# NagabhushanSN95/ViP-NeRF

Measured on AMD Instinct MI355X. Metric: train_rays_per_sec, higher is better.
Workload: dtype f32; 1 GPU; BASELINE configs[1]: fern geometry (NDC), 2 views, 4096 rays/iter/GPU x (64+128) samples, coarse+fine 8x256 MLP, V=1 secondary view(s), losses MSE+Visibility+VisibilityPrior, Adam; rays generated and random numbers drawn on device; rays_per_gpu=4096, global_rays=4096, parallelism=ray-sharded dp1, gemm_arithmetic=fp32

## Files before the change

### vip-nerf_amd/csrc/vipnerf_knobs.h

```cpp
#pragma once

#define VN_KNOB_LIST(X)                                                                                                                   \
                                                    \
    X(VN_BF16_NARROW_DEFAULT) X(VN_FP32_NARROW_DEFAULT)                                                                                   \
                     \
    X(VN_STAGE_CHUNKS) X(VN_SPLIT_FMA_MIX) X(VN_INTERLEAVE) X(VN_SKEW) X(VN_DMA_MODE) X(VN_DMA_ISSUERS) X(VN_F16_PRESPLIT) X(VN_DEFER_STORES)             \
    X(VN_STORE_GROUP_A) X(VN_STORE_GROUP_B) X(VN_F32_PERSISTENT) X(VN_F32_EVAL_ROTATE) X(VN_F32B_CONV_GROUP) X(VN_DMA_ROT_WAVES) X(VN_F32_DMA_ISSUERS)                                                              \
        \
    X(VN_BF16_H16) X(VN_T16) X(VN_T16_X4) X(VN_T16_NT) X(VN_PT2_SPREAD) X(VN_PT2_SKEW) X(VN_PT2_G) X(VN_PT2_D)                  \
    X(VN_PT2_TRAIN_KEEP) X(VN_PT2_EVAL_KEEP) X(VN_PT2_FAST_PE)                                                                                              \
                                                                           \
    X(VN_WGRAD_SIGMA_FUSED) X(VN_WGRAD_VIEW_FUSED) X(VN_WGRAD_HEADS_FUSED) X(VN_WGRAD_LATE_LOAD) X(VN_WGRAD_LATE_STORE) X(VN_WGRAD_STORE_SKEW) X(VN_WGRAD_FAST) X(VN_WGRAD_BIAS_WK0) X(VN_WGRAD_VECFRAG) X(VN_WGRAD_PREFETCH) X(VN_WGRAD_DMA) X(VN_WGRAD_W8) X(VN_WGRAD_PIPE) X(VN_WGRAD_ONE_ROUND) X(VN_WGRAD_ROUNDS) X(VN_WG16_BIG_WM) X(VN_WG16_BIG_WN)        \
    X(VN_WG16_BIG_NB) X(VN_WG16_HYBRID) X(VN_WG16_SIGMA_FUSED) X(VN_WG16_DMA_PIECES) X(VN_WG16_THIN_HYBRID) X(VN_WG16_BIG_SLOTS) X(VN_WG16_VIEW_FUSED) X(VN_WG16_VIEW_WN)          \
                                                                                                         \
    X(VN_ADAM_FMA_MASK)

#ifndef VN_BF16_NARROW_DEFAULT
#define VN_BF16_NARROW_DEFAULT 1
#endif
#ifndef VN_FP32_NARROW_DEFAULT
#define VN_FP32_NARROW_DEFAULT 1
#endif
#ifndef VN_STAGE_CHUNKS
#define VN_STAGE_CHUNKS 64
#endif
#ifndef VN_SPLIT_FMA_MIX
#define VN_SPLIT_FMA_MIX 1
#endif
#ifndef VN_INTERLEAVE
#define VN_INTERLEAVE 1
#endif
#ifndef VN_SKEW
#define VN_SKEW 0
#endif
#ifndef VN_DMA_MODE
#define VN_DMA_MODE 1
#endif
#ifndef VN_DMA_ISSUERS
#define VN_DMA_ISSUERS 1
#endif
#ifndef VN_F16_PRESPLIT
#define VN_F16_PRESPLIT 1
#endif
#ifndef VN_DEFER_STORES
#define VN_DEFER_STORES 1
#endif
#ifndef VN_STORE_GROUP_A
#define VN_STORE_GROUP_A 6
#endif
#ifndef VN_STORE_GROUP_B
#define VN_STORE_GROUP_B 12
#endif
#ifndef VN_F32_PERSISTENT
#define VN_F32_PERSISTENT 1
#endif
#ifndef VN_F32_EVAL_ROTATE
#define VN_F32_EVAL_ROTATE 1
#endif
#ifndef VN_WGRAD_SIGMA_FUSED
#define VN_WGRAD_SIGMA_FUSED 1
#endif
#ifndef VN_WGRAD_VIEW_FUSED
#define VN_WGRAD_VIEW_FUSED 1
#endif
#ifndef VN_F32_DMA_ISSUERS
#define VN_F32_DMA_ISSUERS 4
#endif
#ifndef VN_DMA_ROT_WAVES
#define VN_DMA_ROT_WAVES 4
#endif
#ifndef VN_F32B_CONV_GROUP
#define VN_F32B_CONV_GROUP 2
#endif
#ifndef VN_BF16_H16
#define VN_BF16_H16 1
#endif
#ifndef VN_T16
#define VN_T16 1
#endif
#ifndef VN_T16_X4
#define VN_T16_X4 1
#endif
#ifndef VN_T16_NT
#define VN_T16_NT 1
#endif
#ifndef VN_PT2_SPREAD
#define VN_PT2_SPREAD 4
#endif
#ifndef VN_PT2_SKEW
#define VN_PT2_SKEW 0
#endif
#ifndef VN_PT2_G
#define VN_PT2_G 1
#endif
#ifndef VN_PT2_D
#define VN_PT2_D 2
#endif
#ifndef VN_PT2_TRAIN_KEEP
#define VN_PT2_TRAIN_KEEP 0
#endif
#ifndef VN_PT2_EVAL_KEEP
#define VN_PT2_EVAL_KEEP 1
#endif
#ifndef VN_PT2_FAST_PE
#define VN_PT2_FAST_PE 1
#endif
#ifndef VN_WGRAD_LATE_LOAD
#define VN_WGRAD_LATE_LOAD 2
#endif
#ifndef VN_WGRAD_LATE_STORE
#define VN_WGRAD_LATE_STORE 12
#endif
#ifndef VN_WGRAD_HEADS_FUSED
#define VN_WGRAD_HEADS_FUSED 1
#endif
#ifndef VN_WGRAD_STORE_SKEW
#define VN_WGRAD_STORE_SKEW 2
#endif
#ifndef VN_WGRAD_FAST
#define VN_WGRAD_FAST 1
#endif
#ifndef VN_WGRAD_BIAS_WK0
#define VN_WGRAD_BIAS_WK0 1
#endif
#ifndef VN_WGRAD_VECFRAG
#define VN_WGRAD_VECFRAG 1
#endif
#ifndef VN_WGRAD_PREFETCH
#define VN_WGRAD_PREFETCH 1
#endif
#ifndef VN_WGRAD_DMA
#define VN_WGRAD_DMA 0
#endif
#ifndef VN_WGRAD_W8
#define VN_WGRAD_W8 2
#endif
#ifndef VN_WGRAD_PIPE
#define VN_WGRAD_PIPE 1
#endif
#ifndef VN_WGRAD_ONE_ROUND
#define VN_WGRAD_ONE_ROUND 1
#endif
#ifndef VN_WGRAD_ROUNDS
#define VN_WGRAD_ROUNDS 1
#endif
#ifndef VN_WG16_BIG_WM
#define VN_WG16_BIG_WM 2
#endif
#ifndef VN_WG16_BIG_WN
#define VN_WG16_BIG_WN 4
#endif
#ifndef VN_WG16_BIG_NB
#define VN_WG16_BIG_NB 4
#endif
#ifndef VN_WG16_HYBRID
#define VN_WG16_HYBRID 1
#endif
#ifndef VN_WG16_SIGMA_FUSED
#define VN_WG16_SIGMA_FUSED 1
#endif
#ifndef VN_WG16_DMA_PIECES
#define VN_WG16_DMA_PIECES 2
#endif
#ifndef VN_WG16_THIN_HYBRID
#define VN_WG16_THIN_HYBRID 0
#endif
#ifndef VN_WG16_VIEW_FUSED
#define VN_WG16_VIEW_FUSED 1
#endif
#ifndef VN_WG16_VIEW_WN
#define VN_WG16_VIEW_WN 2
#endif
#ifndef VN_WG16_BIG_SLOTS
#define VN_WG16_BIG_SLOTS 256
#endif
#ifndef VN_ADAM_FMA_MASK
#define VN_ADAM_FMA_MASK 7
#endif

#define VN_KNOB_STR2(x) #x
#define VN_KNOB_STR(x) VN_KNOB_STR2(x)
#define VN_KNOB_ITEM(name) " " #name "=" VN_KNOB_STR(name)
#if defined(VN_EXP)
#define VN_EXP_STR "VN_EXP=" VN_KNOB_STR(VN_EXP)
#define VN_EXP_VALUE (VN_EXP)
#else
#define VN_EXP_STR "VN_EXP=unset"
#define VN_EXP_VALUE (-1)
#endif
#define VN_BUILD_INFO_KNOBS VN_EXP_STR VN_KNOB_LIST(VN_KNOB_ITEM)
```

### vip-nerf_amd/csrc/vipnerf_mlp_fwd_f32.hip

```cpp
#include "vipnerf_bf16n.h"
#include "vipnerf_mlp.h"
#include "vipnerf_mlp_pt2.h"

namespace vn {

TS_DECL(g_f32f_timeline);
#define TSFF(tag) TS_AT(g_f32f_timeline, tag)

typedef BnPlan<2> PLFF;

template <bool SAVE>
__device__ __forceinline__ void fwd_conv_kstep(const floatx4 *xr, f32q (*bin)[2], int s, unsigned *mk, bool sig, float *sg, const float *wsig) {
#pragma unroll
    for (int u = 0; u < 2; ++u) {
        const int t = 2 * s + u;
        floatx4 x;
#pragma unroll
        for (int r = 0; r < 4; ++r) x[r] = SAVE ? relu_bits(xr[t][r], 0) : fmaxf(xr[t][r], 0.f);
        if (SAVE) mk[t >> 3] = push_nibble(mk[t >> 3], positive_nibble(x));
        if (sig) {
            const float4 w4 = *(const float4 *)(wsig + 16 * t);
            sg[0] = fmaf(w4.x, x[0], sg[0]); sg[1] = fmaf(w4.y, x[1], sg[1]);
            sg[2] = fmaf(w4.z, x[2], sg[2]); sg[3] = fmaf(w4.w, x[3], sg[3]);
        }
        bin[s][u].v = x;
    }
}

template <bool SAVE, bool CONV>
struct F32FwdMid {
    float *dst; int64_t p; int q, wave, s0;
    f32q (*bin)[2];
    const floatx4 *xr;
    unsigned *mk;
    bool sig; float *sg; const float *wsig;
    uint2 *mask_dst;
    template <int g, int NG> static constexpr bool active() {
        return (SAVE && (g == VN_STORE_GROUP_A || g == VN_STORE_GROUP_B)) || (CONV && g == VN_F32B_CONV_GROUP);
    }
    template <int g, int NG>
    __device__ __forceinline__ void at() const {
        if (CONV && g == VN_F32B_CONV_GROUP) {
            fwd_conv_kstep<SAVE>(xr, bin, s0 + 2, mk, sig, sg, wsig);
            fwd_conv_kstep<SAVE>(xr, bin, s0 + 3, mk, sig, sg, wsig);
            if (SAVE && s0 == 4 && !EXP_NO_STORES) *mask_dst = make_uint2(mk[0], mk[1]);
        }
        if (SAVE && (g == VN_STORE_GROUP_A || g == VN_STORE_GROUP_B) && (g == VN_STORE_GROUP_A) == (wave < 4) && !EXP_NO_STORES) {
#pragma unroll
            for (int s = s0; s < s0 + 2; ++s) {
                store_tile16(dst, p, W, q, 2 * s, bin[s][0].v);
                store_tile16(dst, p, W, q, 2 * s + 1, bin[s][1].v);
            }
        }
    }
};

template <bool SAVE>
__global__ __launch_bounds__(PLFF::WG) void k_mlp_fwd_f32(MlpFwdArgs a) {
    typedef PLFF PL;
    typedef f32q FR;
    extern __shared__ __attribute__((aligned(16))) float lds[];
    float *res = lds;
    float *stage_buf = lds + PL::R_TOTAL_PAD;
    const float *rf = res + PL::R_F32;

    const int tid = threadIdx.x, lane = tid & 63, wave = tid >> 6;
    const int q = lane >> 4, j = lane & 15;
    const int64_t p_raw = (int64_t)blockIdx.x * MLP_PTS_PER_WG + wave * 16 + j;
    const bool valid = p_raw < a.src.P;
    const int64_t p = valid ? p_raw : a.src.P - 1;

    TS_INIT();
    TSFF(TS_ENTRY);
    typename std::conditional<SAVE || VN_F32_EVAL_ROTATE, typename StreamOlder<PL>::type, typename StreamShared<PL>::type>::type ws;
    ws.start(a.packed + PL::PK_FWD, PL::F_STAGES, stage_buf, lane, wave);
    {
        const float4 *g4 = (const float4 *)(a.packed + PL::PK_RES);
        float4 *l4 = (float4 *)res;
        for (int i = tid; i < PL::R_TOTAL_PAD / 4; i += PL::WG) l4[i] = g4[i];
    }
    float pe[2][8];
    {
        PointCtx pc0;
        load_point(a.src, p, pc0);
        encode_x16(pc0.x, q, pe);
    }
    if (SAVE && valid && !EXP_NO_PE) store_x16(a.acts + a.al.pex + (size_t)p * DPE_PAD, q, pe);
    FR bpe[2][2];
#pragma unroll
    for (int s = 0; s < 2; ++s) split8<2>(pe[s], bpe[s]);

    FR bin[8][2];
    floatx4 acc[16], xr[16];
    unsigned mk[2] = {0u, 0u};
    float sg[4] = {0.f, 0.f, 0.f, 0.f};
    const float *wsig = rf + PL::N_WSIG + 4 * q;

    __syncthreads();
    TSFF(TS_RESIDENT);

    {
        const float *bias = rf + PL::N_BIAS + 4 * q;
#pragma unroll
        for (int t = 0; t < 16; ++t) { const float4 b4 = *(const float4 *)(bias + 16 * t); acc[t][0] = b4.x; acc[t][1] = b4.y; acc[t][2] = b4.z; acc[t][3] = b4.w; }
        TSFF(TS_PRE);
        const float *st = ws.wait();
        TSFF(TS_POST);
        gemm_stage_bf<16, PL::KSB, 2>(st, lane, acc, bpe, 0, ws);
        TSFF(TS_END);
#pragma unroll
        for (int t = 0; t < 16; ++t) xr[t] = acc[t];
    }

#pragma unroll 1
    for (int layer = 1; layer <= 8; ++layer) {
        const float *bias = rf + (layer < 8 ? PL::N_BIAS + layer * W : PL::N_BFEAT) + 4 * q;
#pragma unroll
        for (int t = 0; t < 16; ++t) { const float4 b4 = *(const float4 *)(bias + 16 * t); acc[t][0] = b4.x; acc[t][1] = b4.y; acc[t][2] = b4.z; acc[t][3] = b4.w; }
        TSFF(TS_EPI_A);
        const bool sig = layer == 8;
        float *hdst = SAVE ? a.acts + a.al.h[layer - 1] : nullptr;
        uint2 *mdst = SAVE ? (uint2 *)(a.acts + a.al.hm[layer - 1] + ((size_t)p * 4 + q) * 2) : nullptr;
        mk[0] = 0u; mk[1] = 0u;
        fwd_conv_kstep<SAVE>(xr, bin, 0, mk, sig, sg, wsig);
        fwd_conv_kstep<SAVE>(xr, bin, 1, mk, sig, sg, wsig);
        TSFF(TS_EPI_B);
#pragma unroll
        for (int jj = 0; jj < PL::ST_256; ++jj) {
            TSFF(TS_PRE);
            const float *st = SAVE ? (jj == 0 ? ws.template wait<4, 0>(layer == 1 || layer == 6) : ws.template wait<4>()) : ws.wait();
            TSFF(TS_POST);
            if (jj + 1 < PL::ST_256) {
                F32FwdMid<SAVE, true> mid{hdst, p, q, wave, 2 * jj, bin, xr, mk, sig, sg, wsig, mdst};
                gemm_stage_bf<16, PL::KSB, 2>(st, lane, acc, bin, PL::KSB * jj, ws, mid);
            } else {
                F32FwdMid<SAVE, false> mid{hdst, p, q, wave, 2 * jj, bin, xr, mk, sig, sg, wsig, mdst};
                gemm_stage_bf<16, PL::KSB, 2>(st, lane, acc, bin, PL::KSB * jj, ws, mid);
            }
            TSFF(TS_END);
        }
        if (layer == SKIP_LAYER) {
            TSFF(TS_PRE);
            const float *st = SAVE ? ws.template wait<4>() : ws.wait();
            TSFF(TS_POST);
            gemm_stage_bf<16, PL::KSB, 2>(st, lane, acc, bpe, 0, ws);
            TSFF(TS_END);
        }
#pragma unroll
        for (int t = 0; t < 16; ++t) xr[t] = acc[t];
        TSFF(15);
    }

    {
        float s = (sg[0] + sg[1]) + (sg[2] + sg[3]);
        s += __shfl_xor(s, 16, 64);
        s += __shfl_xor(s, 32, 64);
        const float sigma_raw = s + rf[PL::N_BHEAD];
        float nz = 0.f;
        if (a.ns.noise) nz = a.ns.noise[p];
        else if (a.ns.device_rng) nz = rng_normal(a.ns.seed, a.ns.offset, a.ns.stream, noise_index(a.ns, a.src, p));
        const float sgm = fmaxf(__fadd_rn(sigma_raw, __fmul_rn(nz, a.ns.std)), 0.f);
        if (valid && q == 0) a.sigma[p] = sgm;
    }

#pragma unroll
    for (int s = 0; s < 8; ++s) {
        bin[s][0].v = xr[2 * s]; bin[s][1].v = xr[2 * s + 1];
        if (SAVE && !EXP_NO_EXTRAS) {
            store_tile16(a.acts + a.al.feat, p, W, q, 2 * s, xr[2 * s]);
            store_tile16(a.acts + a.al.feat, p, W, q, 2 * s + 1, xr[2 * s + 1]);
        }
    }
    PointCtx pc;
    load_point(a.src, p, pc);
    floatx4 vb[8];
#pragma unroll
    for (int t = 0; t < 8; ++t) {
        const float4 b4 = *(const float4 *)(rf + PL::N_BVIEW + 16 * t + 4 * q);
        vb[t][0] = b4.x; vb[t][1] = b4.y; vb[t][2] = b4.z; vb[t][3] = b4.w;
    }
#pragma unroll
    for (int jj = 0; jj < PL::ST_VIEW_F; ++jj) {
        TSFF(TS_PRE);
        const float *st = SAVE ? (jj == 0 ? ws.template wait<20>() : ws.template wait<0>()) : ws.wait();
        TSFF(TS_POST);
        gemm_stage_bf<8, PL::KSV, 2>(st, lane, vb, bin, PL::KSV * jj, ws);
        TSFF(TS_VIEW);
    }
    stream_end(ws);
    TSFF(16);

#pragma unroll 1
    for (int dsel = 0; dsel <= a.src.V; ++dsel) {
        float dir[3];
        if (dsel == 0) { dir[0] = pc.dir[0]; dir[1] = pc.dir[1]; dir[2] = pc.dir[2]; }
        else secondary_dir(a.src, pc, dsel - 1, dir);
        TSFF(10);
        float ped[1][8];
        encode_d16(dir, q, ped);
        FR bpd[1][2];
        split8<2>(ped[0], bpd[0]);
        floatx4 g[8];
#pragma unroll
        for (int t = 0; t < 8; ++t) g[t] = vb[t];
        { NoStream none; gemm_stage_bf<8, 1, 2>(res + PL::R_DIRW, lane, g, bpd, 0, none); }
#pragma unroll
        for (int t = 0; t < 8; ++t)
#pragma unroll
            for (int r = 0; r < 4; ++r) g[t][r] = relu_lo<SAVE>(g[t][r], 0.f);
        TSFF(12);
        if (SAVE) {
            if (!EXP_NO_EXTRAS) {
#pragma unroll
                for (int t = 0; t < 8; ++t) store_tile16(a.acts + a.al.g[dsel], p, WV, q, t, g[t]);
                unsigned gmb = 0u;
#pragma unroll
                for (int t = 0; t < 8; ++t) gmb = push_nibble(gmb, positive_nibble(g[t]));
                ((unsigned *)(a.acts + a.al.gm[dsel]))[(size_t)p * 4 + q] = gmb;
            }
            if (valid && !EXP_NO_PE) store_d16(a.acts + a.al.ped[dsel] + (size_t)p * DVE_PAD, q, ped);
        }
        TSFF(13);
        float qv[4];
#pragma unroll
        for (int c = 0; c < 4; ++c) {
            const float *wo = rf + PL::N_WOUT + c * WV + 4 * q;
            float s0 = 0.f, s1 = 0.f;
#pragma unroll
            for (int t = 0; t < 8; ++t) {
                const float4 w4 = *(const float4 *)(wo + 16 * t);
                s0 = fmaf(w4.x, g[t][0], s0);
                s1 = fmaf(w4.y, g[t][1], s1);
                s0 = fmaf(w4.z, g[t][2], s0);
                s1 = fmaf(w4.w, g[t][3], s1);
            }
            float s = s0 + s1;
            s += __shfl_xor(s, 16, 64);
            s += __shfl_xor(s, 32, 64);
            qv[c] = sigmoidf_(s + rf[PL::N_BHEAD + 1 + c]);
        }
        if (valid && q == 0) {
            if (dsel == 0) {
                a.rgb[3 * p + 0] = qv[0]; a.rgb[3 * p + 1] = qv[1]; a.rgb[3 * p + 2] = qv[2];
                a.vis[p] = qv[3];
            } else {
                a.vis2[p * a.src.V + (dsel - 1)] = qv[3];
            }
        }
        TSFF(14);
    }
    TSFF(TS_LAST);
}

#if defined(VN_EXP) && VN_EXP == 50
extern "C" int vipnerf_exp_timeline_f32f(unsigned long long *out, int n) {
    return (int)hipMemcpyFromSymbol(out, HIP_SYMBOL(g_f32f_timeline), sizeof(unsigned long long) * (n < 2048 ? n : 2048));
}
#endif

template <bool SAVE>
static int launch_one_f32(const MlpFwdArgs &a, unsigned grid, hipStream_t st) {
    const size_t lds = (size_t)PLFF::LDS_F * sizeof(float);
    VN_HIP(hipFuncSetAttribute((const void *)k_mlp_fwd_f32<SAVE>, hipFuncAttributeMaxDynamicSharedMemorySize, (int)lds));
    hipLaunchKernelGGL(k_mlp_fwd_f32<SAVE>, dim3(grid), dim3(PLFF::WG), lds, st, a);
    VN_HIP(hipGetLastError());
    return VIPNERF_OK;
}

int launch_mlp_fwd_f32(const MlpFwdArgs &a, hipStream_t st) {
    if (a.src.P <= 0) return VIPNERF_OK;
    const unsigned grid = (unsigned)((a.src.P + MLP_PTS_PER_WG - 1) / MLP_PTS_PER_WG);
    return a.acts ? launch_one_f32<true>(a, grid, st) : launch_one_f32<false>(a, grid, st);
}

}
```

Before: 150,100 rays/s.

## Make f32 MLP forward kernel persistent over tiles and add optional early conversion

The f32 forward MLP kernel now loops over multiple point tiles per workgroup, and the grid is capped at the persistent grid size for the training (SAVE) path. Resident weights are then loaded into LDS once per workgroup instead of once per tile, and the weight stream runs across tiles. An optional, default-off knob moves the ReLU/convert step of each layer's output into the tail of the last GEMM stage. The persistent loop adds per-tile index recomputation and asm barriers to keep register pressure down, and it may reduce parallelism if there are too few tiles.

```diff
diff --git a/vip-nerf_amd/csrc/vipnerf_knobs.h b/vip-nerf_amd/csrc/vipnerf_knobs.h
--- a/vip-nerf_amd/csrc/vipnerf_knobs.h
+++ b/vip-nerf_amd/csrc/vipnerf_knobs.h
@@ -5,7 +5,7 @@
     X(VN_BF16_NARROW_DEFAULT) X(VN_FP32_NARROW_DEFAULT)                                                                                   \
                      \
     X(VN_STAGE_CHUNKS) X(VN_SPLIT_FMA_MIX) X(VN_INTERLEAVE) X(VN_SKEW) X(VN_DMA_MODE) X(VN_DMA_ISSUERS) X(VN_F16_PRESPLIT) X(VN_DEFER_STORES)             \
-    X(VN_STORE_GROUP_A) X(VN_STORE_GROUP_B) X(VN_F32_PERSISTENT) X(VN_F32_EVAL_ROTATE) X(VN_F32B_CONV_GROUP) X(VN_DMA_ROT_WAVES) X(VN_F32_DMA_ISSUERS)                                                              \
+    X(VN_STORE_GROUP_A) X(VN_STORE_GROUP_B) X(VN_F32_PERSISTENT) X(VN_F32_FWD_PERSISTENT) X(VN_F32_EARLY_CONV) X(VN_F32_EVAL_ROTATE) X(VN_F32B_CONV_GROUP) X(VN_DMA_ROT_WAVES) X(VN_F32_DMA_ISSUERS)                                                              \
         \
     X(VN_BF16_H16) X(VN_T16) X(VN_T16_X4) X(VN_T16_NT) X(VN_PT2_SPREAD) X(VN_PT2_SKEW) X(VN_PT2_G) X(VN_PT2_D)                  \
     X(VN_PT2_TRAIN_KEEP) X(VN_PT2_EVAL_KEEP) X(VN_PT2_FAST_PE)                                                                                              \
@@ -53,6 +53,12 @@
 #endif
 #ifndef VN_F32_PERSISTENT
 #define VN_F32_PERSISTENT 1
+#endif
+#ifndef VN_F32_FWD_PERSISTENT
+#define VN_F32_FWD_PERSISTENT 1
+#endif
+#ifndef VN_F32_EARLY_CONV
+#define VN_F32_EARLY_CONV 0
 #endif
 #ifndef VN_F32_EVAL_ROTATE
 #define VN_F32_EVAL_ROTATE 1
diff --git a/vip-nerf_amd/csrc/vipnerf_mlp_fwd_f32.hip b/vip-nerf_amd/csrc/vipnerf_mlp_fwd_f32.hip
--- a/vip-nerf_amd/csrc/vipnerf_mlp_fwd_f32.hip
+++ b/vip-nerf_amd/csrc/vipnerf_mlp_fwd_f32.hip
@@ -56,29 +56,63 @@
 };
 
 template <bool SAVE>
+struct F32FwdTail {
+    const floatx4 *acc;
+    f32q (*bin)[2];
+    unsigned *mk;
+    bool on, sig; float *sg; const float *wsig;
+    template <int g, int NG> static constexpr bool active() { return g > NG / 2; }
+    template <int g, int NG>
+    __device__ __forceinline__ void at() const {
+        static_assert(NG == 16, "a stage of 2 k-steps x 16 tiles in groups of two tiles");
+        if (on) fwd_conv_kstep<SAVE>(acc, bin, g - NG / 2 - 1, mk, sig, sg, wsig);
+    }
+};
+template <typename M1, typename M2>
+struct MidPair {
+    M1 m1; M2 m2;
+    template <int g, int NG> static constexpr bool active() { return M1::template active<g, NG>() || M2::template active<g, NG>(); }
+    template <int g, int NG>
+    __device__ __forceinline__ void at() const {
+        if (M1::template active<g, NG>()) m1.template at<g, NG>();
+        if (M2::template active<g, NG>()) m2.template at<g, NG>();
+    }
+};
+
+template <bool SAVE>
 __global__ __launch_bounds__(PLFF::WG) void k_mlp_fwd_f32(MlpFwdArgs a) {
     typedef PLFF PL;
     typedef f32q FR;
+    constexpr bool EC = VN_F32_EARLY_CONV != 0;
     extern __shared__ __attribute__((aligned(16))) float lds[];
     float *res = lds;
     float *stage_buf = lds + PL::R_TOTAL_PAD;
     const float *rf = res + PL::R_F32;
 
-    const int tid = threadIdx.x, lane = tid & 63, wave = tid >> 6;
-    const int q = lane >> 4, j = lane & 15;
-    const int64_t p_raw = (int64_t)blockIdx.x * MLP_PTS_PER_WG + wave * 16 + j;
-    const bool valid = p_raw < a.src.P;
-    const int64_t p = valid ? p_raw : a.src.P - 1;
+    const int tid = threadIdx.x, wave = __builtin_amdgcn_readfirstlane(tid >> 6);
+    const int64_t n_tiles = (a.src.P + MLP_PTS_PER_WG - 1) / MLP_PTS_PER_WG;
+    const int my_tiles = (int)((n_tiles - blockIdx.x + gridDim.x - 1) / gridDim.x);
 
     TS_INIT();
     TSFF(TS_ENTRY);
     typename std::conditional<SAVE || VN_F32_EVAL_ROTATE, typename StreamOlder<PL>::type, typename StreamShared<PL>::type>::type ws;
-    ws.start(a.packed + PL::PK_FWD, PL::F_STAGES, stage_buf, lane, wave);
+    ws.start(a.packed + PL::PK_FWD, PL::F_STAGES, stage_buf, tid & 63, wave, my_tiles);
     {
         const float4 *g4 = (const float4 *)(a.packed + PL::PK_RES);
         float4 *l4 = (float4 *)res;
         for (int i = tid; i < PL::R_TOTAL_PAD / 4; i += PL::WG) l4[i] = g4[i];
     }
+#pragma unroll 1
+    for (int tile_k = 0; tile_k < my_tiles; ++tile_k) {
+    int lane = tid & 63;
+    asm volatile("" : "+v"(lane));
+    int q = lane >> 4, j = lane & 15;
+    const float *wsig = rf + PL::N_WSIG + 4 * q;
+    int64_t tile_p0 = ((int64_t)blockIdx.x + (int64_t)tile_k * gridDim.x) * MLP_PTS_PER_WG + wave * 16, P = a.src.P;
+    asm volatile("" : "+s"(tile_p0), "+s"(P));
+    bool valid = tile_p0 + j < P;
+    int64_t p = valid ? tile_p0 + j : P - 1;
+
     float pe[2][8];
     {
         PointCtx pc0;
@@ -94,9 +128,8 @@
     floatx4 acc[16], xr[16];
     unsigned mk[2] = {0u, 0u};
     float sg[4] = {0.f, 0.f, 0.f, 0.f};
-    const float *wsig = rf + PL::N_WSIG + 4 * q;
-
-    __syncthreads();
+
+    if (tile_k == 0) __syncthreads();
     TSFF(TS_RESIDENT);
 
     {
@@ -106,32 +139,52 @@
         TSFF(TS_PRE);
         const float *st = ws.wait();
         TSFF(TS_POST);
-        gemm_stage_bf<16, PL::KSB, 2>(st, lane, acc, bpe, 0, ws);
+        if (EC) {
+            F32FwdTail<SAVE> tl{acc, bin, mk, true, false, sg, wsig};
+            gemm_stage_bf<16, PL::KSB, 2>(st, lane, acc, bpe, 0, ws, tl);
+        } else {
+            gemm_stage_bf<16, PL::KSB, 2>(st, lane, acc, bpe, 0, ws);
+        }
         TSFF(TS_END);
-#pragma unroll
-        for (int t = 0; t < 16; ++t) xr[t] = acc[t];
+        if (!EC) {
+#pragma unroll
+            for (int t = 0; t < 16; ++t) xr[t] = acc[t];
+        }
     }
 
 #pragma unroll 1
     for (int layer = 1; layer <= 8; ++layer) {
         const float *bias = rf + (layer < 8 ? PL::N_BIAS + layer * W : PL::N_BFEAT) + 4 * q;
-#pragma unroll
-        for (int t = 0; t < 16; ++t) { const float4 b4 = *(const float4 *)(bias + 16 * t); acc[t][0] = b4.x; acc[t][1] = b4.y; acc[t][2] = b4.z; acc[t][3] = b4.w; }
-        TSFF(TS_EPI_A);
         const bool sig = layer == 8;
         float *hdst = SAVE ? a.acts + a.al.h[layer - 1] : nullptr;
         uint2 *mdst = SAVE ? (uint2 *)(a.acts + a.al.hm[layer - 1] + ((size_t)p * 4 + q) * 2) : nullptr;
-        mk[0] = 0u; mk[1] = 0u;
-        fwd_conv_kstep<SAVE>(xr, bin, 0, mk, sig, sg, wsig);
-        fwd_conv_kstep<SAVE>(xr, bin, 1, mk, sig, sg, wsig);
-        TSFF(TS_EPI_B);
+        if (EC) {
+            fwd_conv_kstep<SAVE>(acc, bin, 7, mk, sig, sg, wsig);
+            if (SAVE && !EXP_NO_STORES) *mdst = make_uint2(mk[0], mk[1]);
+            mk[0] = 0u; mk[1] = 0u;
+#pragma unroll
+            for (int t = 0; t < 16; ++t) { const float4 b4 = *(const float4 *)(bias + 16 * t); acc[t][0] = b4.x; acc[t][1] = b4.y; acc[t][2] = b4.z; acc[t][3] = b4.w; }
+            TSFF(TS_EPI_B);
+        } else {
+#pragma unroll
+            for (int t = 0; t < 16; ++t) { const float4 b4 = *(const float4 *)(bias + 16 * t); acc[t][0] = b4.x; acc[t][1] = b4.y; acc[t][2] = b4.z; acc[t][3] = b4.w; }
+            TSFF(TS_EPI_A);
+            mk[0] = 0u; mk[1] = 0u;
+            fwd_conv_kstep<SAVE>(xr, bin, 0, mk, sig, sg, wsig);
+            fwd_conv_kstep<SAVE>(xr, bin, 1, mk, sig, sg, wsig);
+            TSFF(TS_EPI_B);
+        }
 #pragma unroll
         for (int jj = 0; jj < PL::ST_256; ++jj) {
             TSFF(TS_PRE);
             const float *st = SAVE ? (jj == 0 ? ws.template wait<4, 0>(layer == 1 || layer == 6) : ws.template wait<4>()) : ws.wait();
             TSFF(TS_POST);
             if (jj + 1 < PL::ST_256) {
-                F32FwdMid<SAVE, true> mid{hdst, p, q, wave, 2 * jj, bin, xr, mk, sig, sg, wsig, mdst};
+                F32FwdMid<SAVE, !EC> mid{hdst, p, q, wave, 2 * jj, bin, xr, mk, sig, sg, wsig, mdst};
+                gemm_stage_bf<16, PL::KSB, 2>(st, lane, acc, bin, PL::KSB * jj, ws, mid);
+            } else if (EC) {
+                MidPair<F32FwdMid<SAVE, false>, F32FwdTail<SAVE>> mid{{hdst, p, q, wave, 2 * jj, bin, xr, mk, sig, sg, wsig, mdst},
+                                                                     {acc, bin, mk, layer != SKIP_LAYER && layer < 8, layer + 1 == 8, sg, wsig}};
                 gemm_stage_bf<16, PL::KSB, 2>(st, lane, acc, bin, PL::KSB * jj, ws, mid);
             } else {
                 F32FwdMid<SAVE, false> mid{hdst, p, q, wave, 2 * jj, bin, xr, mk, sig, sg, wsig, mdst};
@@ -143,13 +196,29 @@
             TSFF(TS_PRE);
             const float *st = SAVE ? ws.template wait<4>() : ws.wait();
             TSFF(TS_POST);
-            gemm_stage_bf<16, PL::KSB, 2>(st, lane, acc, bpe, 0, ws);
+            if (EC) {
+                F32FwdTail<SAVE> tl{acc, bin, mk, true, false, sg, wsig};
+                gemm_stage_bf<16, PL::KSB, 2>(st, lane, acc, bpe, 0, ws, tl);
+            } else {
+                gemm_stage_bf<16, PL::KSB, 2>(st, lane, acc, bpe, 0, ws);
+            }
             TSFF(TS_END);
         }
+        if (!EC) {
+#pragma unroll
+            for (int t = 0; t < 16; ++t) xr[t] = acc[t];
+        }
+        TSFF(15);
+    }
+    if (EC) {
 #pragma unroll
         for (int t = 0; t < 16; ++t) xr[t] = acc[t];
-        TSFF(15);
-    }
+    }
+
+    asm volatile("" : "+v"(lane), "+s"(tile_p0), "+s"(P));
+    q = lane >> 4; j = lane & 15;
+    valid = tile_p0 + j < P;
+    p = valid ? tile_p0 + j : P - 1;
 
     {
         float s = (sg[0] + sg[1]) + (sg[2] + sg[3]);
@@ -187,7 +256,6 @@
         gemm_stage_bf<8, PL::KSV, 2>(st, lane, vb, bin, PL::KSV * jj, ws);
         TSFF(TS_VIEW);
     }
-    stream_end(ws);
     TSFF(16);
 
 #pragma unroll 1
@@ -250,6 +318,8 @@
         TSFF(14);
     }
     TSFF(TS_LAST);
+    }
+    stream_end(ws);
 }
 
 #if defined(VN_EXP) && VN_EXP == 50
@@ -269,7 +339,9 @@
 
 int launch_mlp_fwd_f32(const MlpFwdArgs &a, hipStream_t st) {
     if (a.src.P <= 0) return VIPNERF_OK;
-    const unsigned grid = (unsigned)((a.src.P + MLP_PTS_PER_WG - 1) / MLP_PTS_PER_WG);
+    const int64_t tiles = (a.src.P + MLP_PTS_PER_WG - 1) / MLP_PTS_PER_WG;
+    const bool pers = a.acts && VN_F32_FWD_PERSISTENT && tiles > persistent_grid();
+    const unsigned grid = (unsigned)(pers ? persistent_grid() : tiles);
     return a.acts ? launch_one_f32<true>(a, grid, st) : launch_one_f32<false>(a, grid, st);
 }
 
```

After: 150,500 rays/s, median of 6. No clear change (+0.2%).
